# pranavkantgaur/3dscan

Hardware: AMD Instinct MI355X
Metric: Mpixels/s decode+unwrap+triangulate @1920×1080 (higher is better)
Workload: dtype f64

## Files before the change

### 3dscan_amd/__init__.py

```python
__version__ = "0.6.0"
```

### 3dscan_amd/csrc/sl3d_capi_context.cpp

```cpp
#include "sl3d_capi_internal.h"

static thread_local std::string g_create_err;

int sl3d_fail(sl3d_ctx *c, int code, const std::string &msg)
{
    if (c) c->err = msg;
    else g_create_err = msg;
    return code;
}

int sl3d_caught(sl3d_ctx *c, std::string *other) noexcept
{
    int code = SL3D_E_INTERNAL;
    const char *what = "unknown C++ exception";
    char buf[256];
    try {
        throw;
    } catch (const std::bad_alloc &) {
        code = SL3D_E_NOMEM;
        what = "out of host memory (std::bad_alloc)";
    } catch (const std::exception &e) {
        snprintf(buf, sizeof buf, "internal error: %s", e.what());
        what = buf;
    } catch (...) {
    }
    try {
        if (other) *other = what;
        else if (c) c->err = what;
        else g_create_err = what;
    } catch (...) {
    }
    return code;
}
// ... 61 lines not shown

    sl3d_ctx *x = new sl3d_ctx();
    struct Unwind {
        sl3d_ctx *p;
        ~Unwind() { if (p) sl3d_destroy(p); }
    } unwind{x};
    x->cfg = c;
    x->keep = (c.flags & SL3D_FLAG_KEEP_STAGES) != 0;
#define CREATE_CHK(call)                                                                 \
    do {                                                                                 \
        hipError_t e_ = (call);                                                          \
        if (e_ != hipSuccess) {                                                          \
            g_create_err = std::string(#call) + ": " + hipGetErrorString(e_);            \
            return e_ == hipErrorOutOfMemory ? SL3D_E_NOMEM : SL3D_E_HIP;                \
        }                                                                                \
    } while (0)
    DeviceGuard dev_guard_(c.device);
    CREATE_CHK(dev_guard_.err);
    if (c.stream) {
        x->stream = (hipStream_t)c.stream;
    } else {
        CREATE_CHK(hipStreamCreateWithFlags(&x->stream, hipStreamNonBlocking));
        x->own_stream = true;
    }
    CREATE_CHK(hipEventCreate(&x->ev0));
    CREATE_CHK(hipEventCreate(&x->ev1));
    x->lanes_ok = x->own_stream && !(c.flags & (SL3D_FLAG_SERIAL_LAUNCHES | SL3D_FLAG_KEEP_STAGES)) && !getenv("SL3D_NO_LAUNCH_LANES");

    KParams &P = x->P;
    P.W = c.width; P.H = c.height; P.fullW = c.full_width; P.fullH = c.full_height;
    P.col0 = c.col0; P.row0 = c.row0; P.PW = c.proj_width; P.PH = c.proj_height;
    P.F = c.n_fringe; P.Nv = c.n_gray_v; P.Nh = c.n_gray_h; P.fwv = c.fringe_width_v; P.fwh = c.fringe_width_h;
    P.ncodes_v = c.n_codes_v; P.ncodes_h = c.n_codes_h;
#ifdef SL3D_MEASURE
    P.ablate = getenv("SL3D_ABLATE") ? atoi(getenv("SL3D_ABLATE")) : 0;
#endif
    P.pitch = (c.width + 15) & ~15;
    P.planes_per_view = 2 * P.F + 2 * P.Nv + 2 * P.Nh;
    if ((size_t)P.pitch * (size_t)P.H >= ((size_t)1 << 32)) {
        return fail(nullptr, SL3D_E_UNSUPPORTED, "window too large: a plane must stay below 4 GiB (split it into row stripes)");
    }
    P.plane_stride = (size_t)P.pitch * P.H;
    P.view_stride = (size_t)P.planes_per_view * P.plane_stride;
    P.mpitch = P.pitch + 2 * SL3D_MASK_LPAD;
    x->mask_rows = (size_t)P.H + 2 * SL3D_MASK_HALO;
    P.mask_view_stride = (size_t)P.mpitch * x->mask_rows;
    P.px_view_stride = (size_t)P.pitch * P.H;

    if ((P.view_stride >> 32) != 0) {
        g_create_err = "one view's frame stack exceeds 4 GiB: shard the frame by rows";
        return SL3D_E_UNSUPPORTED;
    }
    const size_t V = (size_t)c.max_views;
    int rc;
#define ALLOC(ptr, count)                                              \
    if ((rc = dev_alloc(x, &(ptr), (count))) != SL3D_OK) {             \
        g_create_err = x->err;                                         \
        return rc;                                                     \
    }
    ALLOC(x->d_frames, V * P.view_stride);
    ALLOC(x->d_mask, V * P.mask_view_stride);
    ALLOC(x->d_points, V * P.px_view_stride * 3);
    ALLOC(x->d_valid, V * P.px_view_stride);
    ALLOC(x->d_cal, 1);
    {
        const size_t nb = (P.px_view_stride + 1023) / 1024;
// ... 275 lines not shown
```

### 3dscan_amd/csrc/sl3d_fused.h

```cpp
#pragma once
#include <stddef.h>
#include <stdlib.h>
#include "sl3d_device.h"
#include "sl3d_maskbits.h"

#define SL3D_BLOCK 256
#define SL3D_OCC 4
#define SL3D_SMALL_BLOCK SL3D_BLOCK

#if !defined(SL3D_MEASURE) || !defined(SL3D_ABLATE)
#undef SL3D_ABLATE
#define SL3D_ABLATE 0
#endif
#if defined(SL3D_MEASURE) && defined(SL3D_TRACE)
#define SL3D_STAMP(k)                                                                                                               \
    do {                                                                                                                            \
           \
        if ((CMODE & 2) == 0 && !KEEP && P.dbg)                                                                                           \
            P.dbg[(((size_t)blockIdx.y * gridDim.x + blockIdx.x) * 4 + (threadIdx.x >> 6)) * 8 + (k)] = wall_clock64();              \
    } while (0)
#else
#define SL3D_STAMP(k)
#endif
#ifdef SL3D_MEASURE
#define SL3D_ABLATE_RT(P) ((P).ablate)
#else
#define SL3D_ABLATE_RT(P) 0
#endif

namespace sl3d {


struct PixelResult {
    float x, y, z;
    bool valid;
};

// ... 495 lines not shown
    }
    return vout;
}

template <bool RCP_TAB>
__device__ __forceinline__ void wrapped_quad(int F, const unsigned (&f)[2][4], const double *s_rcp, float (&w)[2][4])
{
    const AtanK AK = atan_consts<true>();
#pragma unroll
    for (int k = 0; k < 4; k++) {
        const int sh = 8 * k;
#pragma unroll
        for (int a = 0; a < 2; a++)
            w[a][k] = shift_pi(wrapped_phase<RCP_TAB>(F, (f[a][0] >> sh) & 255, (f[a][1] >> sh) & 255, (f[a][2] >> sh) & 255, (f[a][3] >> sh) & 255, s_rcp, AK));
    }
}

__device__ __forceinline__ unsigned correspond_quad(const KParams &P, const Item &it, unsigned vbits, const float (&w)[2][4], const unsigned (&code)[2][2], int *my_cp)
{
    unsigned vout = 0;
#pragma unroll
    for (int k = 0; k < 4; k++) {
        const int code_v = (int)((code[0][k >> 1] >> (16 * (k & 1))) & 0xffffu);
        const int code_h = (int)((code[1][k >> 1] >> (16 * (k & 1))) & 0xffffu);
        int cx, cy;
        const bool ok = correspond_px(P, it.gx0 + k, it.gy, w[0][k], w[1][k], code_v, code_h, cx, cy) && ((vbits >> k) & 1u);
        my_cp[3 * k] = ok ? cx : 0;
        my_cp[3 * k + 1] = ok ? cy : 0;
        vout |= (ok ? 1u : 0u) << (8 * k);
    }
    return vout;
}

__device__ __forceinline__ void gather_B(const KParams &P, bool proj_table, const int *my_cp, float2 (&d)[4])
{
#pragma unroll
    for (int k = 0; k < 4; k++) d[k] = make_float2(0.f, 0.f);
    if (proj_table) {
        const GLOBAL_AS uint8_t *tab = opaque((const uint8_t *)P.proj_disp);
        const unsigned pw = (unsigned)P.PW;
#pragma unroll
        for (int k = 0; k < 4; k++) d[k] = ldg_f2(tab, ((unsigned)my_cp[3 * k + 1] * pw + (unsigned)my_cp[3 * k]) * 8u);
    }
}

template <int RIG, bool UNROLL>
__device__ __forceinline__ void phase_B(const KParams &P, const DevCal *Cglobal, const PinnedRows &PR, bool proj_table, unsigned vout, float2 (&d)[4],
                                        const double *my_cam, const int *my_cp, float *my_xyz, const RadEntry *s_rad)
{
    const float nanv = __builtin_nanf("");
    unsigned vb = vout;
#pragma unroll(UNROLL ? 2 : 1)
    for (int j = 0; j < 2; j++) {
        int j8 = j * 8;
        if (!UNROLL) asm volatile("" : "+v"(j8));
        const int pair_words = UNROLL ? 6 * j : ((j8 << 1) + j8) >> 2;
        const int *cp = my_cp + pair_words;
        float *xyz = my_xyz + pair_words;
        const double *cam = my_cam + (UNROLL ? 4 * j : j8 >> 1);
#pragma unroll
        for (int i = 0; i < 2; i++) {
            float x, y, z;
            triangulate_from<RIG>(P, opaque_const(Cglobal), PR, cam[2 * i], cam[2 * i + 1], cp[3 * i], cp[3 * i + 1], d[i], proj_table, s_rad, x, y, z);
            const bool ok = ((vb >> (8 * i)) & 1u) != 0u;
            xyz[3 * i + 0] = ok ? x : nanv;
            xyz[3 * i + 1] = ok ? y : nanv;
// ... 153 lines not shown
template <>
struct RadialLds<3> {
    __device__ __forceinline__ static RadEntry *get()
    {
        __shared__ RadEntry tab[SL3D_RAD_NODES];
        return tab;
    }
};

template <bool KEEP, int NMAX, bool FGEN, bool EXACT, int RIG, int CMODE, bool RCPT, bool EARLY_>
__global__ __launch_bounds__(RCPT ? SL3D_BLOCK : SL3D_SMALL_BLOCK, SL3D_OCC) void k_fused(const KParams P, const DevCal *__restrict__ Cglobal, int first_view, int n_views, int vpt)
{
    constexpr bool SEG = (CMODE & 2) != 0;
    constexpr bool MASKIN = (CMODE & 4) != 0;
    constexpr int BLK = RCPT ? SL3D_BLOCK : SL3D_SMALL_BLOCK;
    static_assert((CMODE & ~6) == 0, "0 = dense planes, 2 = segmented clouds (1 was round 2's look-back compaction), + 4 = MASKIN");
    static_assert(!MASKIN || (!KEEP && RIG != 0 && (RCPT ? !EARLY_ : EARLY_)),
                  "MASKIN: the pipelined small-launch instantiations, and the gated large-launch ones (views known to be sparsely selected)");
    static_assert(!(KEEP && CMODE != 0), "the parity mode writes dense planes");
    static_assert(!(KEEP && RIG != 0), "the parity mode evaluates everything with the reference's operation order");
    __shared__ __attribute__((aligned(16))) float s_xyz[BLK * 12];
    __shared__ __attribute__((aligned(16))) double s_cam[BLK * 8];
    __shared__ __attribute__((aligned(16))) double s_rcp[RCPT ? SL3D_RCP_TAB : 1];
    RadEntry *const s_rad = RadialLds<RIG>::get();
    static_assert(RIG != 3 || SL3D_BLOCK == SL3D_RAD_NODES, "one table node per thread");
    SL3D_STAMP(0);
    constexpr bool PIPE = !KEEP && RIG != 0;
    static_assert(RCPT || EARLY_ == PIPE, "the small-launch instantiation: early requests iff pipelined");
    constexpr bool EARLY = EARLY_ && PIPE;
    constexpr bool REQ_FIRST = PIPE;
    typedef unsigned u32x4 __attribute__((ext_vector_type(4)));
    u32x4 rad_node = {0u, 0u, 0u, 0u};
    if (RIG == 3) rad_node = ((const u32x4 *)P.proj_rad)[(blockIdx.x & 7u) * SL3D_RAD_STRIDE + threadIdx.x];
    if (!REQ_FIRST) {
        if (RIG == 3) ((u32x4 *)s_rad)[threadIdx.x] = rad_node;
        if (RCPT) fill_rcp_table(s_rcp);
        if (RCPT || RIG == 3) __syncthreads();
    }
    SL3D_STAMP(1);
    const int F = FGEN ? P.F : 3;
    float *my_xyz = s_xyz + threadIdx.x * 12;
    double *my_cam = s_cam + threadIdx.x * 8;
    int *my_cp = (int *)my_xyz;
    constexpr bool UNROLL = !RCPT;
#ifdef SL3D_NO_SPLIT
    constexpr bool SPLIT = false;
#else
    constexpr bool SPLIT = EARLY;
#endif

    constexpr int PLANES = EXACT ? 1 : (!KEEP && NMAX <= 12) ? ((MASKIN && RCPT) ? 3 : 2) : 0;
    const int Nv = EXACT ? NMAX : P.Nv, Nh = EXACT ? NMAX : P.Nh;
    const bool proj_table = RIG == 2 || (RIG == 0 && !KEEP && P.proj_disp != nullptr);

    Item it;
    MaskQuad mq;
    double camt[8] = {0, 0, 0, 0, 0, 0, 0, 0};
    unsigned mbits = 0u;
    mrow_t mw0 = {0u, 0u}, mw1 = mw0, mw2 = mw0, mw3 = mw0, mw4 = mw0;
    bool mfast = false;
    unsigned f[2][4], g[2][NMAX], iv[2][NMAX], code[2][2];
    if (!item_begin<RIG, SEG, REQ_FIRST, BLK, MASKIN>(P, Cglobal, blockIdx.x, (int)blockIdx.y, first_view, n_views, vpt, it, mq, camt, my_cam, mw0, mw1, mw2, mw3, mw4, mfast)) return;
    if (MASKIN) it.v_end = it.v_begin + 1;
    if (REQ_FIRST) {
        if (EARLY) {
            issue_fringe<FGEN>(P, it.v_begin, it.lane_off, F, Nv, f);
            issue_gray<NMAX, PLANES>(P, it.v_begin, it.lane_off, F, Nv, Nh, g, iv);
        }
        if (RCPT) fill_rcp_table(s_rcp);
        if (RIG == 3) ((u32x4 *)s_rad)[threadIdx.x] = rad_node;
        if (RCPT || RIG == 3) __syncthreads();
        if (!SEG && !it.alive) return;
        if (MASKIN) {
            if (it.alive) mbits = maskin_finish(P, it, it.v_begin, it.v_begin - first_view, mw0, mw1, mw2, mw3, mw4, mfast);
            maskin_count(P, it, it.v_begin, mbits);
        }
        if (P.use_cam_table) cam_table_finish<RIG, !MASKIN>(P, Cglobal, it, camt, my_cam);
    }
    SL3D_STAMP(2);
    unsigned vb_next = 0;
    if (PIPE) {
        vb_next = MASKIN ? (mbits & 0xfu) : valid_bits<KEEP, FGEN, SEG>(it, F, mq);
        if (!MASKIN && it.v_begin + 1 < it.v_end) mq = load_mask_quad(P, it.v_begin + 1, it.lane_off);
        if (!EARLY && vb_next != 0) {
            issue_fringe<FGEN>(P, it.v_begin, it.lane_off, F, Nv, f);
            issue_gray<NMAX, PLANES>(P, it.v_begin, it.lane_off, F, Nv, Nh, g, iv);
        }
    }
    const PinnedRows PR = pinned_rows<RIG>(Cglobal);
    constexpr bool DEFER = PIPE;
    unsigned pvout = 0;
    auto store_view = [&](int v, unsigned vo) {
        const size_t p = (size_t)v * P.px_view_stride + (size_t)it.lane_off;
        if (MASKIN && it.alive) maskin_store(P, it, v, mbits);
        if (SEG) store_segment(P, it, v, vo, s_xyz, my_xyz);
        else store_quad<KEEP>(P, s_xyz, my_xyz, p, vo);
    };
    for (int view = it.v_begin; view < it.v_end; view++) {
        unsigned vbits;
        if (PIPE) {
            vbits = vb_next;
        } else {
            vbits = valid_bits<KEEP, FGEN, SEG>(it, F, mq);
            if (view + 1 < it.v_end) mq = load_mask_quad(P, view + 1, it.lane_off);
        }
        const size_t px = (size_t)view * P.px_view_stride + (size_t)it.lane_off;
        unsigned vout = 0;
        if (KEEP) parity_init(P, px, vbits);
        if (!DEFER && !SEG && (KEEP || vbits == 0)) fill_nan(my_xyz);
        if (!PIPE && vbits != 0) {
            issue_fringe<FGEN>(P, view, it.lane_off, F, Nv, f);
            issue_gray<NMAX, PLANES>(P, view, it.lane_off, F, Nv, Nh, g, iv);
        }
        if (view == it.v_begin) SL3D_STAMP(3);
        float w[2][4];
        if (SPLIT && vbits != 0) {
            wrapped_quad<RCPT>(F, f, s_rcp, w);
            __builtin_amdgcn_sched_barrier(0);
        }
        if (vbits != 0) decode_gray<NMAX, PLANES>(g, iv, Nv, Nh, code);
        if (view == it.v_begin) SL3D_STAMP(4);
        unsigned vb_pre = 0;
        if (PIPE) {
            vb_pre = MASKIN ? 0u : valid_bits<KEEP, FGEN, SEG>(it, F, mq);
            asm volatile("" : "+v"(vb_pre));
        }
        if (DEFER) {
            if (view > it.v_begin) store_view(view - 1, pvout);
            if (!SEG && vbits == 0) fill_nan(my_xyz);
        }
        if (vbits != 0) {
            if (KEEP) vout = parity_pixels<RCPT>(P, Cglobal, PR, it, F, vbits, f, code, s_rcp, my_cam, my_xyz, px);
            else if (SPLIT) vout = correspond_quad(P, it, vbits, w, code, my_cp);
            else vout = phase_A<RCPT, UNROLL>(P, it, F, vbits, f, code, s_rcp, my_cp);
        }
        if (view == it.v_begin) SL3D_STAMP(5);
        if (PIPE && view + 1 < it.v_end) {
            vb_next = vb_pre;
            if (!MASKIN) mq = load_mask_quad(P, min(view + 2, it.v_end - 1), it.lane_off);
            if (vb_next != 0) {
                issue_fringe<FGEN>(P, view + 1, it.lane_off, F, Nv, f);
                issue_gray<NMAX, PLANES>(P, view + 1, it.lane_off, F, Nv, Nh, g, iv);
            }
        }
        if (!KEEP && vbits != 0) {
            float2 d[4];
            gather_B(P, proj_table, my_cp, d);
            phase_B<RIG, UNROLL>(P, Cglobal, PR, proj_table, vout, d, my_cam, my_cp, my_xyz, s_rad);
        }
        if (DEFER) {
            if (view == it.v_begin) SL3D_STAMP(6);
            pvout = vout;
            continue;
        }
        if (SEG) {
            store_segment(P, it, view, vout, s_xyz, my_xyz);
            continue;
        }
        if (view == it.v_begin) SL3D_STAMP(6);
        store_quad<KEEP>(P, s_xyz, my_xyz, px, vout);
        if (view == it.v_begin) SL3D_STAMP(7);
    }
    if (DEFER) {
        store_view(it.v_end - 1, pvout);
        SL3D_STAMP(7);
// ... 134 lines not shown
```

### 3dscan_amd/csrc/sl3d_fused_launch.hip

```cpp
#include <stdio.h>
#include <stdlib.h>

#include "sl3d_fused.h"

namespace sl3d {

int fused_tiles(const KParams &P)
{
    const long quads = (long)(P.pitch >> 2) * P.H;
    return (int)((quads + SL3D_BLOCK - 1) / SL3D_BLOCK);
}

#define SL3D_VPT_MAX 4
#define SL3D_BLOCK_SLOTS 1024
static int views_per_lane(unsigned bx, int n_views, int cam_table_kind, bool small)
{
    int vpt = 1;
    const int cap = cam_table_kind == 2 ? 8 : SL3D_VPT_MAX;
    const long min_blocks = small ? 4096 : SL3D_BLOCK_SLOTS;
    while (vpt < cap && vpt < n_views && (long)bx * ((n_views + 2 * vpt - 1) / (2 * vpt)) >= min_blocks) vpt *= 2;
#ifdef SL3D_MEASURE
    if (getenv("SL3D_VPT") && atoi(getenv("SL3D_VPT")) >= 1) vpt = atoi(getenv("SL3D_VPT"));
#endif
    return vpt;
}

static int timed_rig(const KParams &P, int rig)
{
    if (P.Nv > 12 || P.Nh > 12 || P.Nv == 0 || P.Nh == 0) return 0;
    return rig == 1 ? 1 : (rig == 2 && P.proj_disp) ? 2 : (rig == 3 && P.proj_rad && P.F == 3) ? 3 : 0;
}

bool fused_maskin_available(const KParams &P, int rig, int n_views, bool keep)
{
    if (keep || P.F != 3 || n_views > SL3D_SMALL_LAUNCH_VIEWS || timed_rig(P, rig) == 0 || (P.cam_tab != nullptr && P.cam_tab_kind == 2)) return false;
    const FusedChoice c = choose_fused(false, false, 0, P.Nv, P.Nh, n_views, false, timed_rig(P, rig));
    return c.small && c.early;
}

unsigned fused_maskin_part_stride(const KParams &P)
{
    const long quads = (long)(P.pitch >> 2) * P.H;
    return 4u * (((unsigned)((quads + SL3D_SMALL_BLOCK - 1) / SL3D_SMALL_BLOCK) + 7u) & ~7u);
}
unsigned fused_maskin_part_words(const KParams &P) { return (unsigned)(((long)(P.pitch >> 2) * P.H + 63) / 64); }

int launch_fused(const KParams &P_, const DevCal *d_cal, int rig, int first_view, int n_views, bool keep, int cmode, void *stream, bool prefer_gated,
                 const MaskIn *mi)
{
    KParams P = P_;
    P.prefer_gated = prefer_gated ? 1 : 0;
    if (mi) {
        if (!fused_maskin_available(P, rig, n_views, keep)) return (int)hipErrorInvalidValue;
        P.mi = *mi;
    }
    const long quads = (long)(P.pitch >> 2) * P.H;
    const unsigned bx = ((unsigned)((quads + SL3D_BLOCK - 1) / SL3D_BLOCK) + 7u) & ~7u;
    const int vpt = mi ? 1 : views_per_lane(bx, n_views, P.cam_tab != nullptr ? P.cam_tab_kind : 0, !keep && P.F == 3 && n_views <= SL3D_SMALL_LAUNCH_VIEWS);
    const dim3 grid(bx, (unsigned)((n_views + vpt - 1) / vpt), 1);
    P.use_cam_table = P.cam_tab != nullptr ? P.cam_tab_kind : 0;
    const int r = timed_rig(P, rig);
#ifdef SL3D_MEASURE
    if (getenv("SL3D_CAMTAB") && atoi(getenv("SL3D_CAMTAB")) == 0) P.use_cam_table = 0;
#endif
    hipStream_t st = (hipStream_t)stream;
    (void)hipGetLastError();
    if (mi) {
        (r == 1 ? fused_maskin_rig1 : r == 2 ? fused_maskin_rig2 : fused_maskin_rig3)(cmode, prefer_gated, P.Nv, P.Nh, grid, st, P, d_cal, first_view, n_views, vpt);
    } else if (keep) {
        fused_parity(P.F != 3, P.Nv, P.Nh, grid, st, P, d_cal, first_view, n_views, vpt);
    } else if (P.F != 3) {
        fused_fgen(r, cmode, P.Nv, P.Nh, grid, st, P, d_cal, first_view, n_views, vpt);
    } else if (cmode == 2) {
        (r == 1 ? fused_clouds_rig1 : r == 2 ? fused_clouds_rig2 : r == 3 ? fused_clouds_rig3 : fused_clouds_rig0)(P.Nv, P.Nh, grid, st, P, d_cal, first_view, n_views, vpt);
    } else {
        (r == 1 ? fused_dense_rig1 : r == 2 ? fused_dense_rig2 : r == 3 ? fused_dense_rig3 : fused_dense_rig0)(P.Nv, P.Nh, grid, st, P, d_cal, first_view, n_views, vpt);
    }
    return (int)hipGetLastError();
}

int fused_kernel_name(const KParams &P, int rig, int n_views, bool keep, int cmode, char *buf, size_t cap, bool prefer_gated, bool maskin)
{
    const bool fgen = P.F != 3;
    const int r = keep ? 0 : timed_rig(P, rig);
    if (maskin) cmode |= 4;
    const FusedChoice c = choose_fused(keep, fgen, cmode & 2, P.Nv, P.Nh, n_views, prefer_gated, r);
    auto b = [](bool v) { return v ? "true" : "false"; };
    return snprintf(buf, cap, "sl3d::k_fused<%s, %d, %s, %s, %d, %d, %s, %s>", b(keep), c.nmax, b(fgen), b(c.exact), r, keep ? 0 : cmode, b(!c.small), b(c.early));
}

}
// ... 1 lines not shown
```

### 3dscan_amd/csrc/sl3d_group.cpp

```cpp
#include <dlfcn.h>
#include <hip/hip_runtime.h>
#include <rccl/rccl.h>

#include <algorithm>
#include <cstdlib>
#include <cstring>
#include <mutex>
#include <string>
#include <vector>

#include "sl3d_ctx.h"

namespace {

struct RcclApi {
    void *lib = nullptr;
    ncclResult_t (*CommInitAll)(ncclComm_t *, int, const int *) = nullptr;
    ncclResult_t (*CommDestroy)(ncclComm_t) = nullptr;
    ncclResult_t (*GroupStart)() = nullptr;
    ncclResult_t (*GroupEnd)() = nullptr;
    ncclResult_t (*Send)(const void *, size_t, ncclDataType_t, int, ncclComm_t, hipStream_t) = nullptr;
    ncclResult_t (*Recv)(void *, size_t, ncclDataType_t, int, ncclComm_t, hipStream_t) = nullptr;
    const char *(*GetErrorString)(ncclResult_t) = nullptr;
    std::string err;
// ... 144 lines not shown
    sl3d_group *g = new sl3d_group();
    g->cfg = *cfg;
    if (g->cfg.full_width == 0) g->cfg.full_width = cfg->width;
    if (g->cfg.full_height == 0) g->cfg.full_height = cfg->height;
    if (g->cfg.max_views <= 0) g->cfg.max_views = 1;
    g->force_rccl = (cfg->flags & SL3D_FLAG_GROUP_FORCE_RCCL) != 0;
    g->distinct_sides = (cfg->flags & SL3D_FLAG_GROUP_DISTINCT_SIDES) != 0;
    const int base = cfg->height / n, rem = cfg->height % n;
    auto bail = [&](int code, const std::string &msg) {
        sl3d_group_destroy(g);
        return gfail(nullptr, code, msg);
    };
    g->st.resize((size_t)n);
    for (int i = 0; i < n; i++) {
        Stripe &s = g->st[(size_t)i];
        s.rows = base + (i < rem ? 1 : 0);
        s.row0 = i * base + std::min(i, rem);
        s.device = devices[i];
        int gi = -1;
        for (size_t k = 0; k < g->gpus.size() && !g->distinct_sides; k++)
            if (g->gpus[k].device == s.device) gi = (int)k;
        if (gi < 0) {
            GpuSide u;
            u.device = s.device;
            g->gpus.push_back(u);
            gi = (int)g->gpus.size() - 1;
        }
        s.gpu = gi;
        sl3d_config c = g->cfg;
        c.height = s.rows;
        c.row0 = g->cfg.row0 + s.row0;
        c.device = s.device;
        c.stream = nullptr;
        c.flags = (cfg->flags & SL3D_FLAG_KEEP_STAGES) | SL3D_FLAG_SERIAL_LAUNCHES;
        const int rc = sl3d_create(&c, &s.ctx);
        if (rc != SL3D_OK) return bail(rc, "stripe " + std::to_string(i) + ": " + sl3d_last_error(nullptr));
        DeviceGuard dg(s.device);
        if (hipEventCreateWithFlags(&s.ev_run, hipEventDisableTiming) != hipSuccess) return bail(SL3D_E_HIP, "hipEventCreate failed");
    }
    for (auto &u : g->gpus) {
        DeviceGuard dg(u.device);
        if (dg.err != hipSuccess || hipStreamCreateWithFlags(&u.comm, hipStreamNonBlocking) != hipSuccess ||
            hipEventCreateWithFlags(&u.ev_comm, hipEventDisableTiming) != hipSuccess)
            return bail(SL3D_E_HIP, "communication stream / event creation failed on device " + std::to_string(u.device));
    }
    const bool wants_rccl = ((g->gpus.size() > 1) || g->force_rccl) && !(cfg->flags & SL3D_FLAG_GROUP_NO_RCCL);
    if (wants_rccl) {
        RcclApi &R = rccl((cfg->flags & SL3D_FLAG_GROUP_DISTINCT_SIDES) != 0);
        if (!R.ok) {
            if (g->force_rccl) return bail(SL3D_E_UNSUPPORTED, "RCCL requested but unavailable: " + R.err);
        } else {
            std::vector<int> devs;
            for (auto &u : g->gpus) devs.push_back(u.device);
            std::vector<ncclComm_t> comms(devs.size(), nullptr);
            (void)hipGetLastError();
            const ncclResult_t r = R.CommInitAll(comms.data(), (int)devs.size(), devs.data());
            if (r != ncclSuccess)
                return bail(SL3D_E_HIP, std::string("ncclCommInitAll: ") + R.GetErrorString(r) +
                                            " (a process that also loads torch must import it BEFORE this library: one ROCm stack per process)");
            for (size_t k = 0; k < devs.size(); k++) g->gpus[k].nccl = comms[k];
            g->use_rccl = true;
        }
    }
    if (!g->use_rccl && g->gpus.size() > 1) {
        DeviceGuard dg(g->gpus[0].device);
        for (size_t k = 1; k < g->gpus.size(); k++) {
            int can = 0;
// ... 380 lines not shown
```

### 3dscan_amd/csrc/sl3d_internal.h

```cpp
#pragma once
#include <stddef.h>
#include <stdint.h>

#include <hip/hip_vector_types.h>

#define SL3D_MASK_HALO 2
#define SL3D_MASK_LPAD 16
#define SL3D_ATAN_T1 511
#define SL3D_ATAN_T2 1021
#define SL3D_MAX_GRAY 16
#define SL3D_SEG_POINTS 256
#define SL3D_SMALL_LAUNCH_VIEWS 4

namespace sl3d {

struct Intr {
    double K[9];
    double ifx, ify, cx, cy;
    double k1, k2, p1, p2, k3;
    int has_dist;
    int affine;
    int has_tan;
    int plain;
    int identity;
// ... 57 lines not shown
    size_t plane_stride;
    size_t view_stride;
    int mpitch;
    size_t mask_view_stride;
    const uint8_t *frames;
    const uint8_t *mask;
    const uint8_t *band;
    const float2 *proj_disp;
    const RadEntry *proj_rad;
    float proj_rad_scale;
    const double *cam_tab;
    int cam_tab_kind;
    int use_cam_table;
    float *points;
    uint8_t *valid;
    size_t px_view_stride;
    float *clouds;
    unsigned long long *cloud_totals;
    int n_tiles;
    int prefer_gated;
    unsigned *seg_counts;
    unsigned long long *seg_offsets;
    int n_segs;
    unsigned long long *dbg;
    float *wrapped[2];
    float *unwrapped[2];
    int32_t *code[2];
    uint8_t *valid_axis[2];
    uint8_t *dbg3[2];
    uint8_t *dbg4[2];
    int64_t *cpmap;
    double *ipoints;
    MaskIn mi;
};
static_assert(SL3D_SMALL_LAUNCH_VIEWS == 4, "KParams::mi_origin holds one entry per view of a small launch");

int launch_fused(const KParams &P, const DevCal *d_cal, int rig, int first_view, int n_views, bool keep, int cmode, void *stream, bool prefer_gated = false,
                 const MaskIn *mi = nullptr);
int fused_kernel_name(const KParams &P, int rig, int n_views, bool keep, int cmode, char *buf, size_t cap, bool prefer_gated = false, bool maskin = false);
bool fused_maskin_available(const KParams &P, int rig, int n_views, bool keep);
unsigned fused_maskin_part_stride(const KParams &P);
unsigned fused_maskin_part_words(const KParams &P);
int launch_seg_scan(const KParams &P, int first_view, int n_views, void *stream);
int launch_seg_close(const KParams &P, int first_view, int n_views, float *dst, size_t dst_view_stride_points, void *stream);
int launch_seg_close_scan(const KParams &P, int first_view, int n_views, float *dst, size_t dst_view_stride_points, unsigned long long capacity_points,
                          void *stream);
int launch_seg_register(const KParams &P, int view, float *out, const float R4[4], float tx, float ty, float tz, void *stream);
int fused_tiles(const KParams &P);
int launch_mask_prepare(const KParams &P, int first_view, int n_views, const MaskSrc &S, unsigned long long *partials, unsigned seq, void *stream);
int mask_prepare_blocks(const KParams &P);
int launch_to_colrow(const KParams &P, int view, int which, void *dst, void *stream);
int launch_mask_from_colrow(const KParams &P, const int *sel, int gx0, int gy0, int ncols, int nrows, uint8_t *raw, void *stream);
int launch_proj_table(const DevCal *d_cal, int PW, int PH, float2 *out, void *stream);
int launch_radial_table(const DevCal *d_cal, int which, double r2max, RadEntry *out, void *stream);
int launch_cam_table(const KParams &P, const DevCal *d_cal, int kind, double *out, void *stream);
int launch_wrap(const KParams &P, int view, int axis, void *stream);
int launch_unwrap(const KParams &P, int view, int axis, void *stream);
int launch_corr(const KParams &P, int view, void *stream);
int launch_tri(const KParams &P, const DevCal &C, int view, void *stream);
int launch_compact(const KParams &P, int view, unsigned *block_counts, unsigned long long *block_offsets, unsigned long long *total,
                   float *cloud, const uint8_t *texture, uint8_t *rgb_out, void *stream);
int launch_compact_views(const KParams &P, int first_view, int n_views, unsigned *block_counts, unsigned long long *block_offsets,
                         unsigned long long *totals, float *clouds, void *stream);
int launch_register(const float *in, float *out, long n, const float R4[4], float tx, float ty, float tz, void *stream);
int launch_synth(const KParams &P, const DevCal &C, const SynthParams &S, int view, void *stream);
int launch_undistort(const uint8_t *src, size_t sstride, uint8_t *dst, size_t dstride, int width, int height, int cn, const double K[9],
// ... 8 lines not shown
```

### 3dscan_amd/scanner.py

```python
import ctypes as C
import os

import numpy as np

_HERE = os.path.dirname(os.path.abspath(__file__))
LIB_PATH = os.environ.get("SL3D_LIB") or os.path.join(_HERE, "libsl3d.so")

SL3D_FLAG_KEEP_STAGES = 1
SL3D_FLAG_GROUP_FORCE_RCCL, SL3D_FLAG_GROUP_NO_RCCL, SL3D_FLAG_GROUP_DISTINCT_SIDES = 2, 4, 16
SL3D_FLAG_EAGER_MASK = 32
SL3D_FLAG_SERIAL_LAUNCHES = 64
AXIS_VERTICAL, AXIS_HORIZONTAL = 0, 1
PATTERN_FRINGE, PATTERN_GRAY, PATTERN_INVERSE_GRAY, PATTERN_BINARY = 0, 1, 2, 3
VALID_VERTICAL, VALID_HORIZONTAL, VALID_MERGED = 0, 1, 2

ABI_SYMBOLS = (
    "sl3d_version", "sl3d_strerror", "sl3d_last_error", "sl3d_create", "sl3d_destroy",
    "sl3d_set_calibration", "sl3d_get_projection_matrices", "sl3d_set_mask", "sl3d_set_masks", "sl3d_set_mask_colrow", "sl3d_set_frames_range", "sl3d_get_global_colrow", "sl3d_set_frames", "sl3d_copy_view", "sl3d_synth_view", "sl3d_get_frames",
    "sl3d_compute_wrapped_phase", "sl3d_unwrap_phase", "sl3d_compute_c_p_map", "sl3d_triangulate",
    "sl3d_run", "sl3d_run_clouds", "sl3d_get_cloud_counts", "sl3d_get_cloud_segments", "sl3d_download_clouds", "sl3d_register_clouds", "sl3d_fused_kernel_name", "sl3d_last_fused_kernel_name", "sl3d_launch_counts", "sl3d_camera_table_bytes_per_pixel", "sl3d_run_timed", "sl3d_synchronize", "sl3d_timer_start", "sl3d_timer_stop",
    "sl3d_get_valid_map", "sl3d_get_wrapped_phase", "sl3d_get_unwrapped_phase", "sl3d_get_code",
    "sl3d_get_debug_image", "sl3d_get_c_p_map", "sl3d_get_intersection_points", "sl3d_get_points",
    "sl3d_get_cloud", "sl3d_set_texture", "sl3d_get_cloud_rgb", "sl3d_compact", "sl3d_compact_views", "sl3d_get_clouds", "sl3d_register_views", "sl3d_transform_cloud", "sl3d_host_alloc", "sl3d_host_free", "sl3d_process_views", "sl3d_undistort", "sl3d_set_frames_raw", "sl3d_pattern_counts", "sl3d_generate_pattern",
    "sl3d_get_device_buffers", "sl3d_download", "sl3d_download_2d",
    "sl3d_group_create", "sl3d_group_destroy", "sl3d_group_last_error", "sl3d_group_size", "sl3d_group_stripe", "sl3d_group_transport",
    "sl3d_group_set_calibration", "sl3d_group_set_mask", "sl3d_group_set_frames", "sl3d_group_run", "sl3d_group_gather",
    "sl3d_group_get_points", "sl3d_group_download_points", "sl3d_group_process_views", "sl3d_group_get_device_buffers", "sl3d_group_run_clouds", "sl3d_group_gather_clouds",
    "sl3d_group_get_cloud", "sl3d_group_synchronize",
)


class Sl3dError(RuntimeError):
    pass


class Config(C.Structure):
    _fields_ = [(n, C.c_int32) for n in (
        "width", "height", "full_width", "full_height", "col0", "row0", "proj_width", "proj_height",
        "n_fringe", "n_gray_v", "n_gray_h", "fringe_width_v", "fringe_width_h", "n_codes_v", "n_codes_h",
        "max_views", "device")] + [("flags", C.c_uint32), ("stream", C.c_void_p)]


class DeviceBuffers(C.Structure):
    _fields_ = [
# ... 102 lines not shown
    L.sl3d_group_transport.argtypes = [vp]
    L.sl3d_group_size.argtypes = [vp]
    L.sl3d_group_stripe.argtypes = [vp, i, C.POINTER(i), C.POINTER(i), C.POINTER(i), C.POINTER(vp)]
    L.sl3d_group_set_calibration.argtypes = [vp] + [vp] * 8
    L.sl3d_group_set_mask.argtypes = [vp, i, vp, C.c_size_t]
    L.sl3d_group_set_frames.argtypes = [vp, i, i, vp, i, C.c_size_t]
    for n in ("sl3d_group_run", "sl3d_group_gather", "sl3d_group_run_clouds"):
        getattr(L, n).argtypes = [vp, i, i]
    L.sl3d_group_gather_clouds.argtypes = [vp, i, i, C.POINTER(C.c_int64)]
    L.sl3d_group_get_points.argtypes = [vp, i, vp, vp]
    L.sl3d_group_download_points.argtypes = [vp, i, i, vp, vp]
    L.sl3d_group_process_views.argtypes = [vp, i, vp, C.c_size_t, vp, vp]
    L.sl3d_group_get_device_buffers.argtypes = [vp, C.POINTER(DeviceBuffers)]
    L.sl3d_group_get_cloud.argtypes = [vp, i, vp, C.c_int64, C.POINTER(C.c_int64)]
    L.sl3d_group_synchronize.argtypes = [vp]
    if path is None:
        _lib = L
    return L


def pattern_counts(proj_extent, fringe_width):
    L = load_library()
    nc, npl = C.c_int(), C.c_int()
    rc = L.sl3d_pattern_counts(proj_extent, fringe_width, C.byref(nc), C.byref(npl))
    if rc != 0:
        raise Sl3dError("sl3d_pattern_counts: " + L.sl3d_strerror(rc).decode())
    return nc.value, npl.value


class Scanner:

    def __init__(self, width, height, proj_width, proj_height, n_gray_v, n_gray_h, fringe_width_v, fringe_width_h,
                 n_fringe=3, n_codes_v=0, n_codes_h=0, max_views=1, device=0, keep_stages=False,
                 full_size=None, origin=(0, 0), stream=None, eager_mask=False, serial_launches=False):
        self.L = load_library()
        fw, fh = full_size if full_size else (width, height)
        self.cfg = Config(width, height, fw, fh, origin[0], origin[1], proj_width, proj_height, n_fringe,
                          n_gray_v, n_gray_h, fringe_width_v, fringe_width_h, n_codes_v, n_codes_h,
                          max_views, device, (SL3D_FLAG_KEEP_STAGES if keep_stages else 0) | (SL3D_FLAG_EAGER_MASK if eager_mask else 0) |
                          (SL3D_FLAG_SERIAL_LAUNCHES if serial_launches else 0), stream)
        self.W, self.H = width, height
        self._h = C.c_void_p()
        rc = self.L.sl3d_create(C.byref(self.cfg), C.byref(self._h))
        if rc != 0:
            raise Sl3dError(f"sl3d_create: {self.L.sl3d_strerror(rc).decode()}: {self.L.sl3d_last_error(None).decode()}")

    def close(self):
        if getattr(self, "_h", None):
            self.L.sl3d_destroy(self._h)
            self._h = None
        for p in getattr(self, "_pinned", []):
            self.L.sl3d_host_free(p)
        self._pinned = []

    def __del__(self):
        try:
            self.close()
        except Exception:
            pass

    def __enter__(self):
        return self

    def __exit__(self, *a):
        self.close()

    def _chk(self, rc, what):
        if rc != 0:
            raise Sl3dError(f"{what}: {self.L.sl3d_strerror(rc).decode()}: {self.L.sl3d_last_error(self._h).decode()}")

    def set_calibration(self, Kc, dc, rc, tc, Kp, dp, rp, tp):
        a = [np.ascontiguousarray(np.asarray(v, dtype=np.float64).ravel()) for v in (Kc, dc, rc, tc, Kp, dp, rp, tp)]
        assert [v.size for v in a] == [9, 5, 3, 3, 9, 5, 3, 3]
# ... 456 lines not shown
```

### include/sl3d.h

```cpp
#ifndef SL3D_H
#define SL3D_H

#include <stddef.h>
#include <stdint.h>

#ifdef __cplusplus
extern "C" {
#endif

#define SL3D_VERSION_STRING "0.6.0"

typedef struct sl3d_ctx sl3d_ctx;

enum sl3d_status {
    SL3D_OK = 0,
    SL3D_E_INVALID_ARG = -1,
    SL3D_E_NO_DEVICE = -2,
    SL3D_E_HIP = -3,
    SL3D_E_STATE = -4,
    SL3D_E_UNSUPPORTED = -5,
    SL3D_E_NOMEM = -6,
    SL3D_E_INTERNAL = -7
};

enum sl3d_axis { SL3D_AXIS_VERTICAL = 0, SL3D_AXIS_HORIZONTAL = 1 };

enum sl3d_valid_which { SL3D_VALID_VERTICAL = 0, SL3D_VALID_HORIZONTAL = 1, SL3D_VALID_MERGED = 2 };

enum sl3d_flags {
    SL3D_FLAG_KEEP_STAGES = 1u,
    SL3D_FLAG_GROUP_FORCE_RCCL = 2u,
    SL3D_FLAG_GROUP_NO_RCCL = 4u,
    SL3D_FLAG_GROUP_DISTINCT_SIDES = 16u,
    SL3D_FLAG_EAGER_MASK = 32u,
    SL3D_FLAG_SERIAL_LAUNCHES = 64u
};

typedef struct sl3d_config {
    int32_t width, height;
    int32_t full_width, full_height;
    int32_t col0, row0;
    int32_t proj_width, proj_height;
    int32_t n_fringe;
    int32_t n_gray_v, n_gray_h;
    int32_t fringe_width_v, fringe_width_h;
    int32_t n_codes_v, n_codes_h;
    int32_t max_views;
    int32_t device;
    uint32_t flags;
    void *stream;
} sl3d_config;

typedef struct sl3d_device_buffers {
    uint8_t *frames;
    size_t frame_pitch;
    size_t plane_stride;
    size_t view_stride;
    int32_t planes_per_view;
    uint8_t *mask;
    size_t mask_pitch;
    size_t mask_view_stride;
    float *points;
    size_t points_pitch;
    size_t points_view_stride;
    uint8_t *valid;
    size_t valid_pitch;
    size_t valid_view_stride;
} sl3d_device_buffers;
// ... 147 lines not shown
```

Measured before the change: 97170.

## Replace per-pixel phase unwrap with host-certified byte-parallel sector lookup

Adds a phase-sector path: when the host can prove, by checking every extreme of the 8-bit fringe lattice for every Gray code, that the rounded unwrapped projector coordinate always equals 2*code plus a sector index, the kernel derives that sector from SWAR byte comparisons of the fringe intensities. This skips the wrapped-phase arctangent, the reciprocal-table fill and its barrier. The proof only succeeds for fringe width 2 with 3 or 4 fringes, and a new EXACT_PHASE flag turns the shortcut off. It also caps views per lane at 2 for large launches when sectors are active, since the per-pixel work is lighter.

```diff
diff --git a/3dscan_amd/__init__.py b/3dscan_amd/__init__.py
--- a/3dscan_amd/__init__.py
+++ b/3dscan_amd/__init__.py
@@ -1 +1 @@
-__version__ = "0.6.0"
+__version__ = "0.7.0"
diff --git a/3dscan_amd/csrc/sl3d_capi_context.cpp b/3dscan_amd/csrc/sl3d_capi_context.cpp
--- a/3dscan_amd/csrc/sl3d_capi_context.cpp
+++ b/3dscan_amd/csrc/sl3d_capi_context.cpp
@@ -1,4 +1,5 @@
 #include "sl3d_capi_internal.h"
+#include "sl3d_phase_sectors.h"
 
 static thread_local std::string g_create_err;
 
@@ -126,6 +127,7 @@
     P.col0 = c.col0; P.row0 = c.row0; P.PW = c.proj_width; P.PH = c.proj_height;
     P.F = c.n_fringe; P.Nv = c.n_gray_v; P.Nh = c.n_gray_h; P.fwv = c.fringe_width_v; P.fwh = c.fringe_width_h;
     P.ncodes_v = c.n_codes_v; P.ncodes_h = c.n_codes_h;
+    P.phase_sectors = !x->keep && !(c.flags & SL3D_FLAG_EXACT_PHASE) && ps_certify(P.F, P.fwv, P.Nv, P.PW, P.fwh, P.Nh, P.PH);
 #ifdef SL3D_MEASURE
     P.ablate = getenv("SL3D_ABLATE") ? atoi(getenv("SL3D_ABLATE")) : 0;
 #endif
diff --git a/3dscan_amd/csrc/sl3d_fused.h b/3dscan_amd/csrc/sl3d_fused.h
--- a/3dscan_amd/csrc/sl3d_fused.h
+++ b/3dscan_amd/csrc/sl3d_fused.h
@@ -3,6 +3,7 @@
 #include <stdlib.h>
 #include "sl3d_device.h"
 #include "sl3d_maskbits.h"
+#include "sl3d_phase_sectors.h"
 
 #define SL3D_BLOCK 256
 #define SL3D_OCC 4
@@ -564,6 +565,27 @@
     return vout;
 }
 
+__device__ __forceinline__ unsigned sector_quad(const KParams &P, const Item &it, int F, unsigned vbits, const unsigned (&f)[2][4], const unsigned (&code)[2][2],
+                                                int *my_cp)
+{
+    const unsigned jv = ps_sector_bytes(F, f[0][0], f[0][1], f[0][2], f[0][3]), jh = ps_sector_bytes(F, f[1][0], f[1][1], f[1][2], f[1][3]);
+    const bool in_h = it.gy >= 1 && it.gy <= P.fullH - 2;
+    unsigned vout = 0;
+#pragma unroll
+    for (int k = 0; k < 4; k++) {
+        const int gx = it.gx0 + k;
+        const bool in_v = gx >= 1 && gx <= P.fullW - 2;
+        const unsigned code_v = (code[0][k >> 1] >> (16 * (k & 1))) & 0xffffu, code_h = (code[1][k >> 1] >> (16 * (k & 1))) & 0xffffu;
+        const unsigned cx = in_v ? 2u * code_v + ((jv >> (8 * k)) & 0xffu) : 0u;
+        const unsigned cy = in_h ? 2u * code_h + ((jh >> (8 * k)) & 0xffu) : 0u;
+        const bool ok = cx < (unsigned)P.PW && cy < (unsigned)P.PH && ((vbits >> k) & 1u);
+        my_cp[3 * k] = ok ? (int)cx : 0;
+        my_cp[3 * k + 1] = ok ? (int)cy : 0;
+        vout |= (ok ? 1u : 0u) << (8 * k);
+    }
+    return vout;
+}
+
 __device__ __forceinline__ void gather_B(const KParams &P, bool proj_table, const int *my_cp, float2 (&d)[4])
 {
 #pragma unroll
@@ -783,10 +805,12 @@
     typedef unsigned u32x4 __attribute__((ext_vector_type(4)));
     u32x4 rad_node = {0u, 0u, 0u, 0u};
     if (RIG == 3) rad_node = ((const u32x4 *)P.proj_rad)[(blockIdx.x & 7u) * SL3D_RAD_STRIDE + threadIdx.x];
+    const bool SECT = !KEEP && P.phase_sectors != 0;
+    const bool RCP_FILL = RCPT && !SECT;
     if (!REQ_FIRST) {
         if (RIG == 3) ((u32x4 *)s_rad)[threadIdx.x] = rad_node;
-        if (RCPT) fill_rcp_table(s_rcp);
-        if (RCPT || RIG == 3) __syncthreads();
+        if (RCP_FILL) fill_rcp_table(s_rcp);
+        if (RCP_FILL || RIG == 3) __syncthreads();
     }
     SL3D_STAMP(1);
     const int F = FGEN ? P.F : 3;
@@ -818,9 +842,9 @@
             issue_fringe<FGEN>(P, it.v_begin, it.lane_off, F, Nv, f);
             issue_gray<NMAX, PLANES>(P, it.v_begin, it.lane_off, F, Nv, Nh, g, iv);
         }
-        if (RCPT) fill_rcp_table(s_rcp);
+        if (RCP_FILL) fill_rcp_table(s_rcp);
         if (RIG == 3) ((u32x4 *)s_rad)[threadIdx.x] = rad_node;
-        if (RCPT || RIG == 3) __syncthreads();
+        if (RCP_FILL || RIG == 3) __syncthreads();
         if (!SEG && !it.alive) return;
         if (MASKIN) {
             if (it.alive) mbits = maskin_finish(P, it, it.v_begin, it.v_begin - first_view, mw0, mw1, mw2, mw3, mw4, mfast);
@@ -865,7 +889,7 @@
         }
         if (view == it.v_begin) SL3D_STAMP(3);
         float w[2][4];
-        if (SPLIT && vbits != 0) {
+        if (SPLIT && vbits != 0 && !SECT) {
             wrapped_quad<RCPT>(F, f, s_rcp, w);
             __builtin_amdgcn_sched_barrier(0);
         }
@@ -882,6 +906,7 @@
         }
         if (vbits != 0) {
             if (KEEP) vout = parity_pixels<RCPT>(P, Cglobal, PR, it, F, vbits, f, code, s_rcp, my_cam, my_xyz, px);
+            else if (SECT) vout = sector_quad(P, it, F, vbits, f, code, my_cp);
             else if (SPLIT) vout = correspond_quad(P, it, vbits, w, code, my_cp);
             else vout = phase_A<RCPT, UNROLL>(P, it, F, vbits, f, code, s_rcp, my_cp);
         }
diff --git a/3dscan_amd/csrc/sl3d_fused_launch.hip b/3dscan_amd/csrc/sl3d_fused_launch.hip
--- a/3dscan_amd/csrc/sl3d_fused_launch.hip
+++ b/3dscan_amd/csrc/sl3d_fused_launch.hip
@@ -13,10 +13,10 @@
 
 #define SL3D_VPT_MAX 4
 #define SL3D_BLOCK_SLOTS 1024
-static int views_per_lane(unsigned bx, int n_views, int cam_table_kind, bool small)
+static int views_per_lane(unsigned bx, int n_views, int cam_table_kind, bool small, bool sectors)
 {
     int vpt = 1;
-    const int cap = cam_table_kind == 2 ? 8 : SL3D_VPT_MAX;
+    const int cap = cam_table_kind == 2 ? 8 : (sectors && !small) ? 2 : SL3D_VPT_MAX;
     const long min_blocks = small ? 4096 : SL3D_BLOCK_SLOTS;
     while (vpt < cap && vpt < n_views && (long)bx * ((n_views + 2 * vpt - 1) / (2 * vpt)) >= min_blocks) vpt *= 2;
 #ifdef SL3D_MEASURE
@@ -56,7 +56,8 @@
     }
     const long quads = (long)(P.pitch >> 2) * P.H;
     const unsigned bx = ((unsigned)((quads + SL3D_BLOCK - 1) / SL3D_BLOCK) + 7u) & ~7u;
-    const int vpt = mi ? 1 : views_per_lane(bx, n_views, P.cam_tab != nullptr ? P.cam_tab_kind : 0, !keep && P.F == 3 && n_views <= SL3D_SMALL_LAUNCH_VIEWS);
+    const int vpt = mi ? 1 : views_per_lane(bx, n_views, P.cam_tab != nullptr ? P.cam_tab_kind : 0, !keep && P.F == 3 && n_views <= SL3D_SMALL_LAUNCH_VIEWS,
+                                        !keep && P.phase_sectors != 0);
     const dim3 grid(bx, (unsigned)((n_views + vpt - 1) / vpt), 1);
     P.use_cam_table = P.cam_tab != nullptr ? P.cam_tab_kind : 0;
     const int r = timed_rig(P, rig);
diff --git a/3dscan_amd/csrc/sl3d_group.cpp b/3dscan_amd/csrc/sl3d_group.cpp
--- a/3dscan_amd/csrc/sl3d_group.cpp
+++ b/3dscan_amd/csrc/sl3d_group.cpp
@@ -200,7 +200,7 @@
         c.row0 = g->cfg.row0 + s.row0;
         c.device = s.device;
         c.stream = nullptr;
-        c.flags = (cfg->flags & SL3D_FLAG_KEEP_STAGES) | SL3D_FLAG_SERIAL_LAUNCHES;
+        c.flags = (cfg->flags & (SL3D_FLAG_KEEP_STAGES | SL3D_FLAG_EXACT_PHASE)) | SL3D_FLAG_SERIAL_LAUNCHES;
         const int rc = sl3d_create(&c, &s.ctx);
         if (rc != SL3D_OK) return bail(rc, "stripe " + std::to_string(i) + ": " + sl3d_last_error(nullptr));
         DeviceGuard dg(s.device);
diff --git a/3dscan_amd/csrc/sl3d_internal.h b/3dscan_amd/csrc/sl3d_internal.h
--- a/3dscan_amd/csrc/sl3d_internal.h
+++ b/3dscan_amd/csrc/sl3d_internal.h
@@ -113,6 +113,7 @@
     int64_t *cpmap;
     double *ipoints;
     MaskIn mi;
+    int phase_sectors;
 };
 static_assert(SL3D_SMALL_LAUNCH_VIEWS == 4, "KParams::mi_origin holds one entry per view of a small launch");
 
diff --git a/3dscan_amd/csrc/sl3d_phase_sectors.h b/3dscan_amd/csrc/sl3d_phase_sectors.h
--- /dev/null
+++ b/3dscan_amd/csrc/sl3d_phase_sectors.h
@@ -0,0 +1,94 @@
+#pragma once
+#include <math.h>
+#include <stdint.h>
+
+#ifdef __HIPCC__
+#define SL3D_PS_FN __host__ __device__ __forceinline__
+#else
+#define SL3D_PS_FN static inline
+#endif
+#define SL3D_PS_HOST static inline
+
+SL3D_PS_FN uint32_t ps_bytes_lt(uint32_t x, uint32_t y)
+{
+    const uint32_t H = 0x80808080u;
+    const uint32_t t = (x | H) - (y & ~H);
+    return ~((x & ~y) | (~(x ^ y) & t)) & H;
+}
+SL3D_PS_FN uint32_t ps_bytes_ceil_avg(uint32_t a, uint32_t b) { return (a | b) - ((a ^ b) >> 1 & 0x7f7f7f7fu); }
+
+SL3D_PS_FN uint32_t ps_sector_bytes(int F, uint32_t p0, uint32_t p1, uint32_t p2, uint32_t p3)
+{
+    const uint32_t n1 = (F == 3 ? ps_bytes_lt(p0, p2) : ps_bytes_lt(p3, p1)) >> 7;
+    const uint32_t n2 = (F == 3 ? ps_bytes_lt(p1, ps_bytes_ceil_avg(p0, p2)) : ps_bytes_lt(p0, p2)) >> 7;
+    return (n2 ^ 0x01010101u) | ((n2 & ~n1) << 1);
+}
+
+#ifndef SL3D_PS_PI
+#define SL3D_PS_PI (22.0 / 7.0)
+#endif
+
+SL3D_PS_HOST double ps_div_exact(double a, double c, double y)
+{
+    const double q0 = a * y;
+    const double r = fma(-q0, c, a);
+    return fma(r, y, q0);
+}
+
+SL3D_PS_HOST double ps_chain(float phi, int code, int fw)
+{
+    const float w = (float)((double)phi + SL3D_PS_PI);
+    const float u = (float)((double)w + ps_div_exact((double)(code * 44), 7.0, 1.0 / 7.0));
+    const double c = 2.0 * SL3D_PS_PI;
+    return rint((double)fw * ps_div_exact((double)u, c, 1.0 / c));
+}
+
+SL3D_PS_HOST float ps_phi(int t1, int t2) { return (float)atan2((double)t1, (double)t2); }
+
+SL3D_PS_HOST int ps_sector(int t1, int t2) { return t2 >= 0 ? 1 : (t1 < 0 ? 0 : 2); }
+
+SL3D_PS_HOST void ps_lattice_extremes(int F, float lo[3], float hi[3])
+{
+    for (int j = 0; j < 3; j++) {
+        lo[j] = INFINITY;
+        hi[j] = -INFINITY;
+    }
+    for (int t1 = -255; t1 <= 255; t1++) {
+        const int a = t1 < 0 ? -t1 : t1;
+        const int m = F == 3 ? 510 - a : 255;
+        const int p = F == 3 ? (a & 1) : 0;
+        const int q = F == 3 ? ((a & 1) ? -1 : -2) : -1;
+        const int ends[4] = {p, m, -m, q};
+        for (int e = 0; e < 4; e++) {
+            const int t2 = ends[e];
+            const int j = ps_sector(t1, t2);
+            const float phi = ps_phi(t1, t2);
+            if (phi < lo[j]) lo[j] = phi;
+            if (phi > hi[j]) hi[j] = phi;
+        }
+    }
+}
+
+SL3D_PS_HOST int ps_certify_axis(const float lo[3], const float hi[3], int fw, int n_gray, int limit)
+{
+    if (fw != 2 || n_gray < 0 || n_gray > 16 || limit < 1) return 0;
+    const double L = (double)(limit - 1);
+    for (int code = 0; code < (1 << n_gray); code++) {
+        for (int j = 0; j < 3; j++) {
+            const double x = (double)(2 * code + j);
+            const double r_lo = ps_chain(lo[j], code, fw), r_hi = ps_chain(hi[j], code, fw);
+            const int same = r_lo == x && r_hi == x;
+            const int both_rejected = x > L && r_lo > L;
+            if (!same && !both_rejected) return 0;
+        }
+    }
+    return 1;
+}
+
+SL3D_PS_HOST int ps_certify(int F, int fw_v, int n_gray_v, int limit_v, int fw_h, int n_gray_h, int limit_h)
+{
+    if (F != 3 && F != 4) return 0;
+    float lo[3], hi[3];
+    ps_lattice_extremes(F, lo, hi);
+    return ps_certify_axis(lo, hi, fw_v, n_gray_v, limit_v) && ps_certify_axis(lo, hi, fw_h, n_gray_h, limit_h);
+}
diff --git a/3dscan_amd/scanner.py b/3dscan_amd/scanner.py
--- a/3dscan_amd/scanner.py
+++ b/3dscan_amd/scanner.py
@@ -10,6 +10,7 @@
 SL3D_FLAG_GROUP_FORCE_RCCL, SL3D_FLAG_GROUP_NO_RCCL, SL3D_FLAG_GROUP_DISTINCT_SIDES = 2, 4, 16
 SL3D_FLAG_EAGER_MASK = 32
 SL3D_FLAG_SERIAL_LAUNCHES = 64
+SL3D_FLAG_EXACT_PHASE = 128
 AXIS_VERTICAL, AXIS_HORIZONTAL = 0, 1
 PATTERN_FRINGE, PATTERN_GRAY, PATTERN_INVERSE_GRAY, PATTERN_BINARY = 0, 1, 2, 3
 VALID_VERTICAL, VALID_HORIZONTAL, VALID_MERGED = 0, 1, 2
@@ -178,13 +179,13 @@
 
     def __init__(self, width, height, proj_width, proj_height, n_gray_v, n_gray_h, fringe_width_v, fringe_width_h,
                  n_fringe=3, n_codes_v=0, n_codes_h=0, max_views=1, device=0, keep_stages=False,
-                 full_size=None, origin=(0, 0), stream=None, eager_mask=False, serial_launches=False):
+                 full_size=None, origin=(0, 0), stream=None, eager_mask=False, serial_launches=False, exact_phase=False):
         self.L = load_library()
         fw, fh = full_size if full_size else (width, height)
         self.cfg = Config(width, height, fw, fh, origin[0], origin[1], proj_width, proj_height, n_fringe,
                           n_gray_v, n_gray_h, fringe_width_v, fringe_width_h, n_codes_v, n_codes_h,
                           max_views, device, (SL3D_FLAG_KEEP_STAGES if keep_stages else 0) | (SL3D_FLAG_EAGER_MASK if eager_mask else 0) |
-                          (SL3D_FLAG_SERIAL_LAUNCHES if serial_launches else 0), stream)
+                          (SL3D_FLAG_SERIAL_LAUNCHES if serial_launches else 0) | (SL3D_FLAG_EXACT_PHASE if exact_phase else 0), stream)
         self.W, self.H = width, height
         self._h = C.c_void_p()
         rc = self.L.sl3d_create(C.byref(self.cfg), C.byref(self._h))
diff --git a/include/sl3d.h b/include/sl3d.h
--- a/include/sl3d.h
+++ b/include/sl3d.h
@@ -8,7 +8,7 @@
 extern "C" {
 #endif
 
-#define SL3D_VERSION_STRING "0.6.0"
+#define SL3D_VERSION_STRING "0.7.0"
 
 typedef struct sl3d_ctx sl3d_ctx;
 
@@ -33,7 +33,8 @@
     SL3D_FLAG_GROUP_NO_RCCL = 4u,
     SL3D_FLAG_GROUP_DISTINCT_SIDES = 16u,
     SL3D_FLAG_EAGER_MASK = 32u,
-    SL3D_FLAG_SERIAL_LAUNCHES = 64u
+    SL3D_FLAG_SERIAL_LAUNCHES = 64u,
+    SL3D_FLAG_EXACT_PHASE = 128u
 };
 
 typedef struct sl3d_config {
```

After: 99910 (median of 6 runs). 2.8% higher.
